# 2gunsu/monocon-pytorch

Hardware: AMD Instinct MI355X
Metric: images/sec (384x1280) fwd+bwd (higher is better)
Workload: dtype f32 (f16x2); 1 GPU; train step B=32/GPU 3x384x1280 (configs[2] shape, fp32 values, mode f16x2); global_batch=32, parallelism=dp1, precision_mode=f16x2

## Files before the change

### monocon-pytorch_amd/csrc/conv_bf16.hip

```cpp
#include "conv_mfma.h"

namespace mc {

typedef __bf16 bf16x8 __attribute__((ext_vector_type(8)));
typedef __bf16 bf16x4 __attribute__((ext_vector_type(4)));
typedef _Float16 f16x8 __attribute__((ext_vector_type(8)));
typedef _Float16 f16x4 __attribute__((ext_vector_type(4)));

template <int SPL> struct Piece { typedef __bf16 T; typedef bf16x8 V8; typedef bf16x4 V4; };
template <> struct Piece<2> { typedef _Float16 T; typedef f16x8 V8; typedef f16x4 V4; };
__device__ __forceinline__ f32x16 mfma_k16(bf16x8 a, bf16x8 b, f32x16 c) { return __builtin_amdgcn_mfma_f32_32x32x16_bf16(a, b, c, 0, 0, 0); }
__device__ __forceinline__ f32x16 mfma_k16(f16x8 a, f16x8 b, f32x16 c) { return __builtin_amdgcn_mfma_f32_32x32x16_f16(a, b, c, 0, 0, 0); }

template <int KS, int S, int WM, int WN, int WTM, int WTN, int SPL>
struct ConvCfgB16 {
    static constexpr int CK = 32;
    static constexpr int PB = WM * WTM, BNT = WN * WTN * 32, NT = 64 * WM * WN;
    static constexpr int KH = win_h(KS), KW = win_w(KS), PAD = win_pad(KS);
    static constexpr int IH = 3 * S + KH, IW = 7 * S + KW, NPIX = IH * IW;
    static constexpr int ROWB = (CK + 8) * 2;
    static constexpr bool PLANAR = S == 1;
    static constexpr int RS = 24;
    static constexpr int PPB = IH * RS * 16;
    static constexpr int CPL = ((PB + 1) / 2) * PPB + 32;
    static_assert(!PLANAR || (2 * IW <= RS && CK == 32), "two patches per 24-slot row, four 16-byte chunks per pixel");
    static constexpr int PLANE_BYTES = PLANAR ? 4 * CPL : PB * NPIX * ROWB;
    static constexpr int TILE_BYTES = SPL * PLANE_BYTES;
    static constexpr size_t LDS_BYTES = TILE_BYTES + PB * 16;
};

template <int KS, int S, int WM, int WN, int WTM, int WTN, int SPL, bool BM = false, bool LZ = false>
__global__ __launch_bounds__(64 * WM * WN, SPL == 1 ? 3 : 2) void conv_bf16_kernel(const ConvArgs a) {
    static_assert(!LZ || (SPL == 2 && !BM), "lazy sources: forward launches of the fp16-split mode");
    using Cfg = ConvCfgB16<KS, S, WM, WN, WTM, WTN, SPL>;
    typedef typename Piece<SPL>::T pc_t;
    typedef typename Piece<SPL>::V8 pc8;
    typedef typename Piece<SPL>::V4 pc4;
    constexpr int PLANE = Cfg::PLANE_BYTES;
    constexpr int CK = Cfg::CK, PB = Cfg::PB, BNT = Cfg::BNT, NT = Cfg::NT, PAD = Cfg::PAD;
    constexpr int IW = Cfg::IW, NPIX = Cfg::NPIX, ROWB = Cfg::ROWB;
    constexpr bool PLANAR = Cfg::PLANAR;
    constexpr int RS = Cfg::RS, PPB = Cfg::PPB, CPL = Cfg::CPL;
    constexpr int C4 = CK / 4;
    static_assert(NT % C4 == 0, "a thread keeps one channel group across its staging elements");

    extern __shared__ __attribute__((aligned(16))) unsigned char lds_raw[];
    int *pinfo = reinterpret_cast<int *>(lds_raw + Cfg::TILE_BYTES);

    const int tid = threadIdx.x;
    const int lane = tid & 63;
    const int wave = __builtin_amdgcn_readfirstlane(tid >> 6);
    const int wm = wave / WN, wn = wave % WN;
    const int g = lane >> 5, li = lane & 31;

    int img, chunk, n0;
    conv_wg<BNT>(a, img, chunk, n0);

    unsigned am_raw[4] = {0u, 0u, 0u, 0u};
    if constexpr (SPL == 2) {
        const int al = lane < AMAX_SUB ? lane * AMAX_STRIDE : 0;
#pragma unroll
        for (int i = 0; i < 4; ++i) am_raw[i] = a.amax_in[i < a.nsrc ? i : 0][al];
    }

    if (tid < PB) {
        const int pp = chunk * PB + tid;
        const int valid = pp < a.ppi;
        const int py = pp / a.ppr, px = pp % a.ppr;
        pinfo[tid * 4 + 0] = img;
        pinfo[tid * 4 + 1] = py * 4;
        pinfo[tid * 4 + 2] = px * 8;
        pinfo[tid * 4 + 3] = valid;
    }
    __syncthreads();

    float a_scale = 1.f, omul = 1.f;
    auto operand_scales = [&] {
        if constexpr (SPL == 2) {
            unsigned v = am_raw[0];
#pragma unroll
            for (int i = 1; i < 4; ++i) v = am_raw[i] > v ? am_raw[i] : v;
            v = lane < AMAX_SUB ? v : 0u;
#pragma unroll
            for (int o = 8; o > 0; o >>= 1) { const unsigned t = (unsigned)__shfl_xor((int)v, o); v = t > v ? t : v; }
            const int ea = f16_scale_exp((unsigned)__builtin_amdgcn_readfirstlane((int)v));
            const int ew = f16_scale_exp(*a.amax_w);
            a_scale = exp2i(ea);
            omul = exp2i(-ea) * exp2i(-ew);
        }
    };
    constexpr int NACC = SPL >= 2 ? 2 : 1;
    f32x16 acc[WTM][WTN], accm[NACC == 2 ? WTM : 1][NACC == 2 ? WTN : 1];
#pragma unroll
    for (int tm = 0; tm < WTM; ++tm)
#pragma unroll
        for (int tn = 0; tn < WTN; ++tn)
#pragma unroll
            for (int r = 0; r < 16; ++r) {
                acc[tm][tn][r] = 0.f;
                if (NACC == 2) accm[tm][tn][r] = 0.f;
            }

    constexpr int TOTAL = PB * NPIX * C4;
    constexpr int NIT = (TOTAL + NT - 1) / NT;
    const int c4 = tid % C4;
    unsigned char *stage_dst = lds_raw + (tid / C4) * ROWB + c4 * 8;

    int a_off[WTM];
#pragma unroll
    for (int tm = 0; tm < WTM; ++tm) {
        const int p = wm * WTM + tm;
        a_off[tm] = PLANAR ? g * CPL + (p >> 1) * PPB + ((li >> 3) * RS + (li & 7) + IW * (p & 1)) * 16
                           : (p * NPIX + ((li >> 3) * S) * IW + (li & 7) * S) * ROWB + g * 16;
    }

    const int Cin8 = a.Cin >> 3;
    const int w_plane = Cfg::KH * Cfg::KW * a.Cin * a.CoutP * 2;
    const __amdgpu_buffer_rsrc_t r_w = make_rsrc(a.wpk16, (unsigned)(SPL * w_plane));
    const int w_lane = (g * a.CoutP + n0 + wn * WTN * 32 + li) * 16;

    constexpr int KSTEPS = CK / 16, NS = Cfg::KH * Cfg::KW * KSTEPS;
    auto load_b = [&](pc8(&dst)[SPL][WTN], int kc, int s) {
        const int tap = s / KSTEPS, m = s % KSTEPS;
        const int soff = (tap * Cin8 + ((kc + m * 16) >> 3)) * a.CoutP * 16;
#pragma unroll
        for (int q = 0; q < SPL; ++q)
#pragma unroll
            for (int tn = 0; tn < WTN; ++tn)
                dst[q][tn] = __builtin_bit_cast(
                    pc8, __builtin_amdgcn_raw_buffer_load_b128(r_w, w_lane + tn * 32 * 16, soff + q * w_plane, 0));
    };
    auto load_a = [&](pc8(&dst)[SPL][WTM], int s) {
        const int tap = s / KSTEPS, m = s % KSTEPS;
#pragma unroll
        for (int q = 0; q < SPL; ++q)
#pragma unroll
            for (int tm = 0; tm < WTM; ++tm)
                dst[q][tm] = *reinterpret_cast<const pc8 *>(
                    lds_raw + q * PLANE + a_off[tm] +
                    (PLANAR ? 2 * m * CPL + ((tap / Cfg::KW) * RS + (tap % Cfg::KW)) * 16
                            : ((tap / Cfg::KW) * IW + (tap % Cfg::KW)) * ROWB + m * 32));
    };
#ifndef MC_CONV_DB_REGS
#define MC_CONV_DB_REGS 48
#endif
    constexpr int DB_FIT = MC_CONV_DB_REGS / (SPL * WTN * 4);
    constexpr int DB = (WTM * WTN > 2) ? 2 : ((DB_FIT >= 6 && NS % 6 == 0) ? 6 : ((DB_FIT >= 3 && NS % 3 == 0) ? 3 : 2));
    static_assert(NS % DB == 0, "ring slots must line up across K-chunks");
    pc8 bq[DB][SPL][WTN];
#pragma unroll
    for (int j = 0; j < DB - 1; ++j) load_b(bq[j], 0, j);
    const EpiCoef<WTN> coef = conv_epi_coef<WN, WTN, BM>(a, n0, wn, li);

#ifndef MC_CONV_PF
#define MC_CONV_PF 1
#endif
    constexpr bool PF = MC_CONV_PF && NIT <= 8 && WTM * WTN <= 2;
    constexpr int UB = NIT > 8 ? 8 : NIT;
    f32x4 pv[PF ? NIT : 1];
    int voff[NIT], sdst[NIT];
    int si = 0, c0 = 0, kc = 0;
    int Cs = a.src[0].C;
    f32x4 lzA = {0.f, 0.f, 0.f, 0.f}, lzB = lzA;
    bool lz_cur = false, lz_next = false;
    auto lazy_fetch = [&](int s_idx, int cc0) {
        if constexpr (LZ) {
            lz_next = a.src[s_idx].la != nullptr;
            if (lz_next) {
                lzA = reinterpret_cast<const f32x4 *>(a.src[s_idx].la + cc0)[c4];
                lzB = reinterpret_cast<const f32x4 *>(a.src[s_idx].lb + cc0)[c4];
            }
        }
    };
    auto lazy_advance = [&] {
        if constexpr (LZ) {
            lz_cur = lz_next;
            if (lz_cur) {
#pragma unroll
                for (int j = 0; j < 4; ++j) { lzA[j] *= a_scale; lzB[j] *= a_scale; }
            }
        }
    };
    __amdgpu_buffer_rsrc_t r_in = make_rsrc(a.src[0].p + (size_t)img * a.Hin * a.Win * Cs, (unsigned)(a.Hin * a.Win * Cs) * 4u);
    auto lane_offsets = [&](int cs) {
#pragma unroll
        for (int i = 0; i < NIT; ++i) {
            const int e = tid + NT * i;
            const int t = e / C4;
            const int pix = t % NPIX;
            const int p = (t / NPIX) % PB;
            const int iy = pix / IW, ix = pix % IW;
            const int y = pinfo[p * 4 + 1] * S - PAD + iy;
            const int x = pinfo[p * 4 + 2] * S - PAD + ix;
            const bool ok = (e < TOTAL) & (pinfo[p * 4 + 3] != 0) & ((unsigned)y < (unsigned)a.Hin) & ((unsigned)x < (unsigned)a.Win);
            int off = ((y * a.Win + x) * cs + c4 * 4) * 4;
            asm volatile("" : "+v"(off));
            voff[i] = ok ? off : BUF_OOB;
            sdst[i] = PLANAR ? (c4 >> 1) * CPL + (p >> 1) * PPB + (iy * RS + ix + IW * (p & 1)) * 16 + (c4 & 1) * 8
                             : (int)(stage_dst - lds_raw) + i * (NT / C4) * ROWB;
        }
    };
    auto stage_load = [&](__amdgpu_buffer_rsrc_t r, int vo, int so) -> f32x4 { return buf_load4(r, vo, so); };
    auto stage_one = [&](const f32x4 &v, int i, auto lz_c) {
        constexpr bool LZC = decltype(lz_c)::value;
        if (i < NIT && (NT * (i + 1) <= TOTAL || tid + NT * i < TOTAL)) {
            pc4 q[SPL];
            [[maybe_unused]] const float cap = voff[i] != BUF_OOB ? __builtin_inff() : 0.f;
#pragma unroll
            for (int j = 0; j < 4; ++j) {
                float r = SPL == 2 ? (LZC ? lazy_act(v[j], lzA[j], lzB[j], cap) : v[j] * a_scale) : v[j];
#pragma unroll
                for (int pz = 0; pz < SPL; ++pz) {
                    q[pz][j] = (pc_t)r;
                    r -= (float)q[pz][j];
                }
            }
#pragma unroll
            for (int pz = 0; pz < SPL; ++pz) *reinterpret_cast<pc4 *>(lds_raw + sdst[i] + pz * PLANE) = q[pz];
        }
    };
#ifdef MC_PHASE_TIMERS
    unsigned long long tp_stage = 0, tp_bar = 0, tp_mfma = 0, tp_epi = 0;
    const unsigned long long tp_t0 = __builtin_readcyclecounter();
#define TP_NOW() __builtin_readcyclecounter()
#else
#define TP_NOW() 0ull
#endif
    lane_offsets(Cs);
    lazy_fetch(0, 0);
    if (PF) {
#pragma unroll
        for (int i = 0; i < NIT; ++i) pv[i] = stage_load(r_in, voff[i], 0);
    }
    __builtin_amdgcn_sched_barrier(0);
    operand_scales();
    for (bool first = true;; first = false) {
        [[maybe_unused]] unsigned long long tp_a = TP_NOW();
        if (!first) __syncthreads();
        [[maybe_unused]] unsigned long long tp_b = TP_NOW();
        lazy_advance();
        auto stage_chunk = [&](auto lz_c) {
            if (PF) {
#pragma unroll
                for (int i = 0; i < NIT; ++i) stage_one(pv[i], i, lz_c);
            } else {
#pragma unroll
                for (int i0 = 0; i0 < NIT; i0 += UB) {
                    f32x4 v[UB];
#pragma unroll
                    for (int u = 0; u < UB; ++u)
                        if (i0 + u < NIT) v[u] = stage_load(r_in, voff[i0 + u], c0 * 4);
#pragma unroll
                    for (int u = 0; u < UB; ++u) stage_one(v[u], i0 + u, lz_c);
                }
            }
        };
        if constexpr (LZ) {
            if (lz_cur) stage_chunk(std::true_type{});
            else stage_chunk(std::false_type{});
        } else {
            stage_chunk(std::false_type{});
        }
        [[maybe_unused]] unsigned long long tp_c = TP_NOW();
        __syncthreads();
        [[maybe_unused]] unsigned long long tp_d = TP_NOW();
        int nsi = si, nc0 = c0 + CK;
        if (nc0 >= Cs) { ++nsi; nc0 = 0; }
        const bool more = nsi < a.nsrc;
        if (more && nsi != si) {
            Cs = a.src[nsi].C;
            r_in = make_rsrc(a.src[nsi].p + (size_t)img * a.Hin * a.Win * Cs, (unsigned)(a.Hin * a.Win * Cs) * 4u);
            lane_offsets(Cs);
        }
        if (more) lazy_fetch(nsi, nc0);
        if (PF && more) {
#pragma unroll
            for (int i = 0; i < NIT; ++i) pv[i] = stage_load(r_in, voff[i], nc0 * 4);
        }
        {
            const int kc_next = (kc + CK < a.Cin) ? kc + CK : kc;
            pc8 acur[SPL][WTM];
            load_a(acur, 0);
#pragma unroll
            for (int s = 0; s < NS; ++s) {
                pc8 anext[SPL][WTM];
                if (s + 1 < NS) load_a(anext, s + 1);
                {
                    const int t = s + DB - 1;
                    if (t < NS) load_b(bq[t % DB], kc, t);
                    else load_b(bq[t % DB], kc_next, t - NS);
                }
                __builtin_amdgcn_sched_barrier(0);
                constexpr int NP = SPL == 1 ? 1 : (SPL == 2 ? 3 : 6);
                constexpr int PA[6] = {SPL == 2 ? 1 : 0, SPL == 2 ? 0 : 2, SPL == 2 ? 0 : 1, 0, 1, 0};
                constexpr int PBv[6] = {SPL == 2 ? 0 : 2, SPL == 2 ? 1 : 0, SPL == 2 ? 0 : 1, 1, 0, 0};
#pragma unroll
                for (int pp = 0; pp < NP; ++pp)
#pragma unroll
                    for (int tm = 0; tm < WTM; ++tm)
#pragma unroll
                        for (int tn = 0; tn < WTN; ++tn) {
                            if (NACC == 2 && pp < NP - 1)
                                accm[tm][tn] = mfma_k16(acur[PA[pp]][tm], bq[s % DB][PBv[pp]][tn], accm[tm][tn]);
                            else
                                acc[tm][tn] = mfma_k16(acur[SPL == 1 ? 0 : PA[pp]][tm], bq[s % DB][SPL == 1 ? 0 : PBv[pp]][tn], acc[tm][tn]);
                        }
                if (s + 1 < NS) {
#pragma unroll
                    for (int q = 0; q < SPL; ++q)
#pragma unroll
                        for (int tm = 0; tm < WTM; ++tm) acur[q][tm] = anext[q][tm];
                }
            }
        }
#ifdef MC_PHASE_TIMERS
        { const unsigned long long tp_e = TP_NOW(); tp_bar += (tp_b - tp_a) + (tp_d - tp_c); tp_stage += tp_c - tp_b; tp_mfma += tp_e - tp_d; }
#endif
        if (!more) break;
        si = nsi; c0 = nc0; kc += CK;
    }
    [[maybe_unused]] const unsigned long long tp_f = TP_NOW();

    if (NACC == 2) {
#pragma unroll
        for (int tm = 0; tm < WTM; ++tm)
#pragma unroll
            for (int tn = 0; tn < WTN; ++tn)
#pragma unroll
                for (int r = 0; r < 16; ++r) acc[tm][tn][r] += accm[tm][tn][r];
    }
    conv_epilogue<WM, WN, WTM, WTN, BNT, BM>(a, acc, pinfo, chunk * PB, img, n0, wm, wn, g, li, coef, omul);
#ifdef MC_PHASE_TIMERS
    if (a.phase_prof && lane == 0) {
        __builtin_amdgcn_s_waitcnt(0);
        const unsigned long long tp_g = TP_NOW();
        tp_epi = tp_g - tp_f;
        unsigned long long *o = a.phase_prof + ((size_t)blockIdx.x * (NT / 64) + wave) * 5;
        o[0] = tp_stage; o[1] = tp_bar; o[2] = tp_mfma; o[3] = tp_epi; o[4] = tp_g - tp_t0;
    }
#endif
}

template <int KS, int S, class Sh, int SPL, bool BM = false, bool LZ = false>
static hipError_t launch_b16_one(ConvArgs a, hipStream_t st, ConvArgs *resolved) {
    using Cfg = ConvCfgB16<KS, S, Sh::WM, Sh::WN, Sh::WTM, Sh::WTN, SPL>;
    static_assert(Cfg::PB == Sh::PB && Cfg::BNT == Sh::BNT, "the shape table and the kernel agree on the tile");
    if constexpr (!LZ) {
        if (conv_any_lazy(a)) {
            if constexpr (SPL == 2 && !BM && (KS == 3 || KS == 1)) {
                if (a.bm_y) return hipErrorInvalidValue;
                return launch_b16_one<KS, S, Sh, SPL, false, true>(a, st, resolved);
            } else {
                return hipErrorInvalidValue;
            }
        }
    }
    if constexpr (!BM && S == 1 && (KS == 3 || KS == 1)) {
        if (a.bm_y) return launch_b16_one<KS, S, Sh, SPL, true>(a, st, resolved);
    } else if constexpr (!BM) {
        if (a.bm_y) return hipErrorInvalidValue;
    }
    conv_set_patches(a, Cfg::PB);
    if (a.CoutP % Cfg::BNT) return hipErrorInvalidValue;
    if (resolved) *resolved = a;
    return launch_dyn_lds<conv_bf16_kernel<KS, S, Sh::WM, Sh::WN, Sh::WTM, Sh::WTN, SPL, BM, LZ>>(
        Cfg::LDS_BYTES, dim3((unsigned)(a.B * a.chunks * (a.CoutP / Cfg::BNT))), dim3(Cfg::NT), st, a);
}

bool conv_bf16_ok(const ConvArgs &a, int ks, int stride) {
    if (!a.wpk16) return false;
    if (a.prec == 3) {
        if (!a.amax_w) return false;
        for (int i = 0; i < a.nsrc; ++i)
            if (!a.amax_in[i]) return false;
    }
    for (int i = 0; i < a.nsrc; ++i)
        if (a.src[i].C % 32) return false;
    if (ks == 3) return stride == 1 || stride == 2;
    return stride == 1 && (ks == 1 || ks == 12 || ks == 21 || ks == 22);
}

template <int SPL>
static hipError_t launch_conv_b16_spl(const ConvArgs &a, int ks, int stride, hipStream_t st, ConvArgs *resolved) {
    return with_conv_window(ks, stride, [&](auto win) {
        return with_conv_shape(a.cfg, [&](auto sh) {
            return launch_b16_one<decltype(win)::KS, decltype(win)::S, decltype(sh), SPL>(a, st, resolved);
        });
    });
}

hipError_t launch_conv_bf16(const ConvArgs &a, int ks, int stride, hipStream_t st, ConvArgs *resolved) {
    if (!conv_bf16_ok(a, ks, stride)) return hipErrorInvalidValue;
    if (a.prec == 3) return launch_conv_b16_spl<2>(a, ks, stride, st, resolved);
    return a.prec == 2 ? launch_conv_b16_spl<3>(a, ks, stride, st, resolved) : launch_conv_b16_spl<1>(a, ks, stride, st, resolved);
}

}
```

### monocon-pytorch_amd/csrc/conv_mfma.h

```cpp
#pragma once
#include <hip/hip_runtime.h>
#include <stdint.h>
#include <atomic>
#include <type_traits>
#include <utility>

namespace mc {

typedef float f32x16 __attribute__((ext_vector_type(16)));
typedef float f32x4 __attribute__((ext_vector_type(4)));

struct DynLdsOnce {
    std::atomic<unsigned long long> done{0};
    hipError_t ensure(const void *fn, int bytes) {
        int dev = 0;
        if (hipGetDevice(&dev) != hipSuccess || dev < 0 || dev >= 64) return hipFuncSetAttribute(fn, hipFuncAttributeMaxDynamicSharedMemorySize, bytes);
        if ((done.load(std::memory_order_acquire) >> dev) & 1ull) return hipSuccess;
        const hipError_t e = hipFuncSetAttribute(fn, hipFuncAttributeMaxDynamicSharedMemorySize, bytes);
        if (e == hipSuccess) done.fetch_or(1ull << dev, std::memory_order_release);
        return e;
    }
};

struct ConvSrc {
    const float *p;
    int C;
    const float *la, *lb;
};
__device__ __forceinline__ float lazy_act(float y, float a, float b, float cap) {
    return __builtin_amdgcn_fmed3f(__builtin_fmaf(y, a, b), 0.f, cap);
}

struct ConvArgs {
    ConvSrc src[4];
    int nsrc;
    int B, Hin, Win, Hout, Wout;
    int Cin;
    int Cout, CoutP;
    const float *wpk;
    const float *scale;
    const float *bias;
    const float *res;
    int res_ld;
    float *out;
    int out_ld, out_coff;
    int relu;
    float *stats;
    const float *stat_shift;
    int stats_centred;
    int ppr, ppi, chunks;
    int cfg;
    int o_img, o_row, o_px, r_img, r_row, r_px;
    const void *wpk16;
    int prec;
    const float *bm_y;
    const float *bm_z;
    const unsigned *bm_zbits;
    const float *bm_a, *bm_b;
    int bm_relu;
    const unsigned *amax_in[4];
    const unsigned *amax_w;
    unsigned *amax_out;
    unsigned long long *phase_prof;
};

__host__ __device__ __forceinline__ int f16_scale_exp(unsigned amax_bits) {
    const int E = (int)((amax_bits >> 23) & 0xffu);
    if (E == 0) return 0;
    const int e = 141 - E;
    return e > 126 ? 126 : e;
}
__host__ __device__ __forceinline__ float exp2i(int e) {
    const unsigned u = (unsigned)(127 + e) << 23;
    return __builtin_bit_cast(float, u);
}
constexpr int AMAX_SUB = 16, AMAX_STRIDE = 64, AMAX_WORDS = AMAX_SUB * AMAX_STRIDE;
__device__ __forceinline__ void amax_commit(unsigned *slot, unsigned bits) {
    unsigned *p = slot + (blockIdx.x % AMAX_SUB) * AMAX_STRIDE;
    if (bits < 0x7f800000u && bits > __hip_atomic_load(p, __ATOMIC_RELAXED, __HIP_MEMORY_SCOPE_AGENT)) atomicMax(p, bits);
}
__device__ __forceinline__ void amax_update_block(unsigned *slot, float v) {
    __shared__ unsigned s_amax;
    if (threadIdx.x == 0) s_amax = 0u;
    __syncthreads();
    const unsigned bits = __builtin_bit_cast(unsigned, v);
    if (bits < 0x7f800000u && bits != 0u) atomicMax(&s_amax, bits);
    __syncthreads();
    if (threadIdx.x == 0) amax_commit(slot, s_amax);
}
__device__ __forceinline__ void amax_update_wave(unsigned *slot, float v) {
#pragma unroll
    for (int o = 32; o > 0; o >>= 1) v = fmaxf(v, __shfl_xor(v, o));
    if ((threadIdx.x & 63) == 0) amax_commit(slot, __builtin_bit_cast(unsigned, v));
}
__device__ __forceinline__ unsigned amax_read(const unsigned *slot) {
    const int lane = threadIdx.x & 63;
    unsigned v = lane < AMAX_SUB ? slot[lane * AMAX_STRIDE] : 0u;
#pragma unroll
    for (int o = 8; o > 0; o >>= 1) { const unsigned t = (unsigned)__shfl_xor((int)v, o); v = t > v ? t : v; }
    return (unsigned)__builtin_amdgcn_readfirstlane((int)v);
}

constexpr int win_h(int ks) { return ks >= 10 ? ks / 10 : ks; }
constexpr int win_w(int ks) { return ks >= 10 ? ks % 10 : ks; }
constexpr int win_pad(int ks) { return ks == 3 ? 1 : 0; }

template <int KS, int S, int CK, int WM, int WN, int WTM, int WTN>
struct ConvCfg {
    static constexpr int PB = WM * WTM;
    static constexpr int BNT = WN * WTN * 32;
    static constexpr int NT = 64 * WM * WN;
    static constexpr int KH = win_h(KS), KW = win_w(KS);
    static constexpr int PAD = win_pad(KS);
    static constexpr int IH = 3 * S + KH;
    static constexpr int IW = 7 * S + KW;
    static constexpr int NPIX = IH * IW;
    static constexpr int CKP = CK + 4;
    static constexpr int LDS_FLOATS = PB * NPIX * CKP + PB * 4;
    static constexpr size_t LDS_BYTES = sizeof(float) * LDS_FLOATS;
};

constexpr int BUF_OOB = (int)0x80000000;
typedef int i32x4 __attribute__((ext_vector_type(4)));
__device__ __forceinline__ __amdgpu_buffer_rsrc_t make_rsrc(const void *base, unsigned bytes) {
    return __builtin_amdgcn_make_buffer_rsrc(const_cast<void *>(base), 0, (int)bytes, 0x00020000);
}
__device__ __forceinline__ f32x4 buf_load4(__amdgpu_buffer_rsrc_t r, int voff, int soff) {
    return __builtin_bit_cast(f32x4, __builtin_amdgcn_raw_buffer_load_b128(r, voff, soff, 0));
}
__device__ __forceinline__ float buf_load1(__amdgpu_buffer_rsrc_t r, int voff, int soff) {
    return __builtin_bit_cast(float, __builtin_amdgcn_raw_buffer_load_b32(r, voff, soff, 0));
}
__device__ __forceinline__ void buf_store1(float v, __amdgpu_buffer_rsrc_t r, int voff, int soff) {
    __builtin_amdgcn_raw_buffer_store_b32(__builtin_bit_cast(int, v), r, voff, soff, 0);
}

#ifndef MC_XCD_ORDER
#define MC_XCD_ORDER 1
#endif
__device__ __forceinline__ int xcd_order(int b, int n) {
    if (!MC_XCD_ORDER) return b;
    const int xcd = b & 7, idx = b >> 3, q = n >> 3, r = n & 7;
    return (xcd < r ? xcd * (q + 1) : r * (q + 1) + (xcd - r) * q) + idx;
}

template <int BNT>
__device__ __forceinline__ void conv_wg(const ConvArgs &a, int &img, int &chunk, int &n0) {
    const int ntiles = a.CoutP / BNT;
    const int bid = xcd_order(blockIdx.x, gridDim.x);
    const int nt = bid % ntiles;
    const int mchunk = bid / ntiles;
    img = mchunk / a.chunks, chunk = mchunk % a.chunks;
    n0 = nt * BNT;
}

template <int WTN>
struct EpiCoef {
    float sc[WTN], bi[WTN], sh[WTN], ma[WTN], mb[WTN];
};
template <int WN, int WTN, bool BM>
__device__ __forceinline__ EpiCoef<WTN> conv_epi_coef(const ConvArgs &a, int n0, int wn, int li) {
    EpiCoef<WTN> c;
#pragma unroll
    for (int tn = 0; tn < WTN; ++tn) {
        const int n = n0 + (wn * WTN + tn) * 32 + li;
        const bool nok = n < a.Cout;
        c.sc[tn] = (a.scale && nok) ? a.scale[n] : 1.f;
        c.bi[tn] = (a.bias && nok) ? a.bias[n] : 0.f;
        c.sh[tn] = (a.stat_shift && nok) ? a.stat_shift[n] : 0.f;
        c.ma[tn] = (BM && a.bm_relu == 2 && nok) ? a.bm_a[n] : 0.f;
        c.mb[tn] = (BM && a.bm_relu == 2 && nok) ? a.bm_b[n] : 0.f;
    }
    return c;
}

template <int WM, int WN, int WTM, int WTN, int BNT, bool BM = false>
__device__ __forceinline__ void conv_epilogue(const ConvArgs &a, f32x16 (&acc)[WTM][WTN], const int *pinfo,
                                              int patch0, int img, int n0, int wm, int wn, int g, int li,
                                              const EpiCoef<WTN> &coef, float omul = 1.f, float *vmax_acc = nullptr) {
#pragma clang fp contract(off)
    const bool do_stats = a.stats != nullptr;
    float vmax = 0.f;
    const bool has_res = a.res != nullptr;
    constexpr bool bm = BM;
    const int bm_relu = a.bm_relu;
    const float floor_v = a.relu ? 0.f : -__builtin_inff();
    const __amdgpu_buffer_rsrc_t r_out = make_rsrc(a.out + (size_t)img * a.o_img, (unsigned)a.o_img * 4u);
    const __amdgpu_buffer_rsrc_t r_res =
        make_rsrc(has_res ? a.res + (size_t)img * a.r_img : a.out, has_res ? (unsigned)a.r_img * 4u : 0u);
    const __amdgpu_buffer_rsrc_t r_y = make_rsrc(bm ? a.bm_y + (size_t)img * a.o_img : a.out, bm ? (unsigned)a.o_img * 4u : 0u);
    const bool zbits = bm && bm_relu == 1 && a.bm_zbits != nullptr;
    const int zwords = a.Cout >> 5;
    const unsigned zimg = zbits ? (unsigned)(a.Hout * a.Wout * zwords) * 4u : (unsigned)a.o_img * 4u;
    const __amdgpu_buffer_rsrc_t r_z =
        make_rsrc(bm && bm_relu == 1 ? (zbits ? reinterpret_cast<const float *>(a.bm_zbits) + (size_t)img * a.Hout * a.Wout * zwords
                                              : a.bm_z + (size_t)img * a.o_img)
                                     : a.out,
                  bm && bm_relu == 1 ? zimg : 0u);
#pragma unroll
    for (int tn = 0; tn < WTN; ++tn) {
        const int n = n0 + (wn * WTN + tn) * 32 + li;
        const bool nok = n < a.Cout;
        const float sc = coef.sc[tn] * omul, bi = coef.bi[tn], sh = coef.sh[tn], ma = coef.ma[tn], mb = coef.mb[tn];
        const int v_out = nok ? (4 * g * a.o_px + a.out_coff + n) * 4 : BUF_OOB;
        const int v_res = nok ? (4 * g * a.r_px + n) * 4 : BUF_OOB;
        const int v_bm = nok ? (4 * g * a.o_px + n) * 4 : BUF_OOB;
        const int v_zb = nok ? (4 * g * zwords + (n >> 5)) * 4 : BUF_OOB;
#pragma unroll
        for (int tm = 0; tm < WTM; ++tm) {
            const int p = wm * WTM + tm;
            const int oy0 = __builtin_amdgcn_readfirstlane(pinfo[p * 4 + 1]);
            const int ox0 = __builtin_amdgcn_readfirstlane(pinfo[p * 4 + 2]);
            const int pv = __builtin_amdgcn_readfirstlane(pinfo[p * 4 + 3]);
            if (!pv) continue;
            float ssum = 0.f, ssq = 0.f;
            if (oy0 + 4 <= a.Hout && ox0 + 8 <= a.Wout) {
                const int s_out = (oy0 * a.o_row + ox0 * a.o_px) * 4;
                const int s_res = (oy0 * a.r_row + ox0 * a.r_px) * 4;
                auto body = [&](auto res_c, auto zmask_c) {
                    constexpr bool RES = decltype(res_c)::value, ZMASK = decltype(zmask_c)::value;
                    float rv[16], yv[16], zv[16];
                    if constexpr (RES) {
#pragma unroll
                        for (int r = 0; r < 16; ++r)
                            rv[r] = buf_load1(r_res, v_res, s_res + ((r >> 2) * a.r_row + (r & 3) * a.r_px) * 4);
                    }
                    if constexpr (bm) {
#pragma unroll
                        for (int r = 0; r < 16; ++r)
                            yv[r] = buf_load1(r_y, v_bm, s_out + ((r >> 2) * a.o_row + (r & 3) * a.o_px) * 4);
                        if constexpr (ZMASK) {
                            if (zbits) {
                                const int s_zb = (oy0 * a.Wout + ox0) * zwords * 4;
#pragma unroll
                                for (int r = 0; r < 16; ++r) {
                                    const unsigned w = __builtin_bit_cast(unsigned, buf_load1(r_z, v_zb, s_zb + ((r >> 2) * a.Wout + (r & 3)) * zwords * 4));
                                    zv[r] = ((w >> (n & 31)) & 1u) ? 1.f : 0.f;
                                }
                            } else {
#pragma unroll
                                for (int r = 0; r < 16; ++r)
                                    zv[r] = buf_load1(r_z, v_bm, s_out + ((r >> 2) * a.o_row + (r & 3) * a.o_px) * 4);
                            }
                        }
                    }
#pragma unroll
                    for (int r = 0; r < 16; ++r) {
                        float v = __builtin_fmaf(acc[tm][tn][r], sc, bi);
                        if constexpr (RES) v += rv[r];
                        if constexpr (bm) {
                            const bool on = ZMASK ? zv[r] > 0.f : (bm_relu == 0 || fmaf(yv[r], ma, mb) > 0.f);
                            v = on ? v : 0.f;
                            ssum += v;
                            ssq = fmaf(v, yv[r], ssq);
                        } else if (do_stats) {
                            const float d = v - sh;
                            ssum += d;
                            ssq += d * d;
                        }
                        v = fmaxf(v, floor_v);
                        vmax = fmaxf(vmax, fabsf(v));
                        buf_store1(v, r_out, v_out, s_out + ((r >> 2) * a.o_row + (r & 3) * a.o_px) * 4);
                    }
                };
                using T = std::true_type;
                using Fz = std::false_type;
                const bool zmask = bm && bm_relu == 1;
                if (has_res) { if (zmask) body(T{}, T{}); else body(T{}, Fz{}); }
                else { if (zmask) body(Fz{}, T{}); else body(Fz{}, Fz{}); }
            } else {
#pragma unroll
                for (int r = 0; r < 16; ++r) {
                    const int y = oy0 + (r >> 2), x = ox0 + (r & 3) + 4 * g;
                    if (nok && y < a.Hout && x < a.Wout) {
                        float v = __builtin_fmaf(acc[tm][tn][r], sc, bi);
                        if (has_res) v += buf_load1(r_res, (y * a.r_row + x * a.r_px + n) * 4, 0);
                        if (bm) {
                            const float yy = buf_load1(r_y, (y * a.o_row + x * a.o_px + n) * 4, 0);
                            bool on = true;
                            if (bm_relu == 1)
                                on = zbits ? ((__builtin_bit_cast(unsigned, buf_load1(r_z, ((y * a.Wout + x) * zwords + (n >> 5)) * 4, 0)) >> (n & 31)) & 1u) != 0u
                                           : buf_load1(r_z, (y * a.o_row + x * a.o_px + n) * 4, 0) > 0.f;
                            else if (bm_relu == 2) on = fmaf(yy, ma, mb) > 0.f;
                            v = on ? v : 0.f;
                            ssum += v;
                            ssq = fmaf(v, yy, ssq);
                        } else {
                            const float d = v - sh;
                            ssum += d;
                            ssq += d * d;
                        }
                        v = fmaxf(v, floor_v);
                        vmax = fmaxf(vmax, fabsf(v));
                        buf_store1(v, r_out, (y * a.o_row + x * a.o_px + a.out_coff + n) * 4, 0);
                    }
                }
            }
            if (do_stats) {
                ssum += __shfl_xor(ssum, 32);
                if constexpr (!bm) {
                    if (a.stats_centred) {
                        const float m = ssum * 0.03125f;
                        ssq = 0.f;
#pragma unroll
                        for (int r = 0; r < 16; ++r) {
                            const float e = (__builtin_fmaf(acc[tm][tn][r], sc, bi) - sh) - m;
                            ssq = __builtin_fmaf(e, e, ssq);
                        }
                    }
                }
                ssq += __shfl_xor(ssq, 32);
                if (g == 0 && nok) {
                    float *dst = a.stats + (((size_t)img * a.ppi + patch0 + p) * a.CoutP + n) * 2;
                    dst[0] = ssum;
                    dst[1] = ssq;
                }
            }
        }
    }
    if (vmax_acc) *vmax_acc = fmaxf(*vmax_acc, vmax);
    else if (a.amax_out) amax_update_wave(a.amax_out, vmax);
}

enum ConvCfgId {
    CFG_AUTO = 0,
    CFG_128x128 = 1,
    CFG_128x64 = 4,
    CFG_128x64m = 5,
    CFG_128x32 = 6,
    CFG_64x128 = 7,
    CFG_64x64 = 8,
    CFG_SHAPE_BITS = 15,
    CFG_WS = 16,
    CFG_SMALL = 32,
    CFG_WRES = 64
};
struct ConvShape {
    int id, WM, WN, WTM, WTN;
    constexpr int PB() const { return WM * WTM; }
    constexpr int BNT() const { return WN * WTN * 32; }
};
constexpr ConvShape CONV_SHAPES[] = {
    {CFG_128x128, 2, 2, 2, 2}, {CFG_128x64, 2, 2, 2, 1}, {CFG_128x64m, 4, 1, 1, 2},
    {CFG_128x32, 4, 1, 1, 1},  {CFG_64x128, 1, 4, 2, 1}, {CFG_64x64, 2, 2, 1, 1},
};
constexpr int CONV_NSHAPES = (int)(sizeof(CONV_SHAPES) / sizeof(CONV_SHAPES[0]));
inline ConvShape conv_shape(int cfg) {
    for (const ConvShape &s : CONV_SHAPES)
        if (s.id == (cfg & CFG_SHAPE_BITS)) return s;
    return {0, 0, 0, 0, 0};
}
// ... 91 lines not shown
```

### monocon-pytorch_amd/csrc/mc_api.hip

```cpp
#include <hip/hip_runtime.h>

#include <algorithm>
#include <cmath>
#include <cstdarg>
#include <cstdio>
#include <cstring>
#include <cstdlib>
#include <map>
#include <memory>
#include <string>
#include <unordered_map>
#include <vector>

#include "../../include/monocon_hip.h"
#include "conv_mfma.h"
#include "kernels.h"

#include <cstdint>
#include "mc_internal.h"

std::string g_create_err;

float *PlanAlloc::alloc(size_t nfloats) {
    const size_t bytes = (nfloats ? nfloats : empty_floats) * sizeof(float);
// ... 922 lines not shown

int mc_op_stem_dgrad_fused(mc_handle *h, const float *d_nhwc, const float *y_nhwc, const float *coef, const float *weight_oihw,
                           int B, int H, int W, float *dx_nchw, void *stream) {
    if (!h) return -1;
    if (!d_nhwc || !y_nhwc || !coef || !weight_oihw || !dx_nchw) return fail(h, "mc_op_stem_dgrad_fused: null argument");
    if (B < 1 || H < 1 || W < 1) return fail(h, "mc_op_stem_dgrad_fused: B, H, W must be >= 1 (got %d, %d, %d)", B, H, W);
    if (reinterpret_cast<uintptr_t>(d_nhwc) % 16 || reinterpret_cast<uintptr_t>(y_nhwc) % 16 || reinterpret_cast<uintptr_t>(coef) % 16)
        return fail(h, "mc_op_stem_dgrad_fused: d_nhwc, y_nhwc and coef must be 16-byte aligned");
    HIPCHK(h, hipSetDevice(h->device));
    HIPCHK(h, launch_stem_dgrad(d_nhwc, weight_oihw, B, H, W, dx_nchw, static_cast<hipStream_t>(stream), y_nhwc, coef));
    return 0;
}

int mc_op_maxpool2(mc_handle *h, const float *in, int B, int H, int W, int C, float *out, void *stream) {
    if (!h) return -1;
    if (!in || !out || (C % 4) || (H % 2) || (W % 2)) return fail(h, "mc_op_maxpool2: bad argument");
    HIPCHK(h, hipSetDevice(h->device));
    HIPCHK(h, launch_maxpool2(in, B, H, W, C, out, static_cast<hipStream_t>(stream)));
    return 0;
}

int mc_op_deconv4x4(mc_handle *h, const float *in, int B, int H, int W, int C, const float *weight, float *out,
                    void *stream) {
    if (!h) return -1;
    if (!in || !out || !weight || (C % 4)) return fail(h, "mc_op_deconv4x4: bad argument");
    HIPCHK(h, hipSetDevice(h->device));
    hipStream_t st = static_cast<hipStream_t>(stream);
    ScratchBuf wpk;
    HIPCHK(h, wpk.alloc((size_t)16 * C * sizeof(float)));
    HIPCHK(h, launch_pack_deconv_w(weight, C, wpk.as<float>(), st));
    hipError_t e = launch_deconv4(in, B, H, W, C, wpk.as<float>(), out, st);
    hipError_t e2 = hipStreamSynchronize(st);
    HIPCHK(h, e);
    HIPCHK(h, e2);
    return 0;
}

int mc_op_nchw_to_nhwc(mc_handle *h, const float *in, int B, int C, int H, int W, float *out, void *stream) {
    if (!h) return -1;
    if (!in || !out) return fail(h, "mc_op_nchw_to_nhwc: null argument");
    HIPCHK(h, hipSetDevice(h->device));
    HIPCHK(h, launch_nchw_to_nhwc(in, B, C, H, W, out, static_cast<hipStream_t>(stream)));
    return 0;
}

int mc_op_nhwc_to_nchw(mc_handle *h, const float *in, int B, int C, int H, int W, float *out, void *stream) {
    if (!h) return -1;
    if (!in || !out) return fail(h, "mc_op_nhwc_to_nchw: null argument");
    HIPCHK(h, hipSetDevice(h->device));
    HIPCHK(h, launch_nhwc_to_nchw(in, B, C, H, W, out, static_cast<hipStream_t>(stream)));
    return 0;
}

int mc_preprocess(mc_handle *h, const void *img_hwc, int dtype, int H, int W, const double mean[3], const double std[3],
                  int pad_h, int pad_w, float *out_chw, void *stream) {
    if (!h) return -1;
    if (!img_hwc || !mean || !std || !out_chw) return fail(h, "mc_preprocess: null argument");
    if (dtype != 0 && dtype != 2) return fail(h, "mc_preprocess: dtype must be 0 (float32) or 2 (uint8)");
    if (H < 1 || W < 1 || pad_h < H || pad_w < W) return fail(h, "mc_preprocess: bad shape %dx%d -> %dx%d", H, W, pad_h, pad_w);
    for (int c = 0; c < 3; ++c)
        if (std[c] == 0.0) return fail(h, "mc_preprocess: std[%d] is zero", c);
    HIPCHK(h, hipSetDevice(h->device));
    HIPCHK(h, launch_preprocess(img_hwc, dtype == 2, H, W, mean, std, pad_h, pad_w, out_chw, static_cast<hipStream_t>(stream)));
    return 0;
}

int mc_preprocess_augmented(mc_handle *h, const unsigned char *frames_hwc, const float *params, int B, int src_h, int src_w,
                            const double mean[3], const double std[3], int pad_h, int pad_w, float *out_bchw, void *stream) {
    if (!h) return -1;
    if (!frames_hwc || !params || !mean || !std || !out_bchw) return fail(h, "mc_preprocess_augmented: null argument");
    if (B < 1 || src_h < 1 || src_w < 1 || pad_h < 1 || pad_w < 1 || B > 65535 || pad_h > 65535)
        return fail(h, "mc_preprocess_augmented: bad shape B=%d %dx%d -> %dx%d", B, src_h, src_w, pad_h, pad_w);
    for (int c = 0; c < 3; ++c)
        if (std[c] == 0.0) return fail(h, "mc_preprocess_augmented: std[%d] is zero", c);
    HIPCHK(h, hipSetDevice(h->device));
    HIPCHK(h, launch_preprocess_aug(frames_hwc, params, B, src_h, src_w, mean, std, pad_h, pad_w, out_bchw, static_cast<hipStream_t>(stream)));
    return 0;
}

int mc_bench_mfma_peak(mc_handle *h, int waves_per_simd, int iters, float *tflops) {
    if (!h || !tflops) return fail(h, "mc_bench_mfma_peak: null argument");
    HIPCHK(h, hipSetDevice(h->device));
    void *out = nullptr;
    HIPCHK(h, hipMalloc(&out, 64));
    hipEvent_t e0, e1;
    HIPCHK(h, hipEventCreate(&e0));
    HIPCHK(h, hipEventCreate(&e1));
    const int blocks = 256 * (waves_per_simd < 0 ? -waves_per_simd : waves_per_simd);
    hipLaunchKernelGGL(mfma_peak_kernel, dim3(blocks), dim3(256), 0, nullptr, (float *)out, 100, waves_per_simd < 0 ? -1.0f : 1.0f);
    (void)hipEventRecord(e0, nullptr);
    hipLaunchKernelGGL(mfma_peak_kernel, dim3(blocks), dim3(256), 0, nullptr, (float *)out, iters, waves_per_simd < 0 ? -1.0f : 1.0f);
    (void)hipEventRecord(e1, nullptr);
    (void)hipEventSynchronize(e1);
    float ms = 0;
    (void)hipEventElapsedTime(&ms, e0, e1);
    *tflops = (float)((double)blocks * 4 * iters * 16 * 4096.0 / (ms * 1e-3) / 1e12);
    (void)hipEventDestroy(e0);
    (void)hipEventDestroy(e1);
    (void)hipFree(out);
    return 0;
}

int mc_bench_conv(mc_handle *h, int B, int Hin, int Win, int nsrc, const int src_channels[], int Cout, int ksize,
                  int stride, int cfg, int iters, float *ms_avg) {
    if (!h || !src_channels || !ms_avg) return fail(h, "mc_bench_conv: null argument");
    HIPCHK(h, hipSetDevice(h->device));
    ConvArgs a{};
    std::vector<void *> bufs;
    const bool zero_data = std::getenv("MONOCON_BENCH_ZERO") != nullptr;
    auto alloc_fill = [&](size_t n, float scale) -> float * {
        if (zero_data) scale = 0.f;
        void *q = nullptr;
        if (hipMalloc(&q, n * sizeof(float)) != hipSuccess) return nullptr;
        bufs.push_back(q);
        std::vector<float> hst(std::min<size_t>(n, (size_t)1 << 22));
        unsigned s = 12345u + (unsigned)bufs.size();
        for (auto &v : hst) { s = s * 1664525u + 1013904223u; v = scale * (((s >> 8) & 0xFFFF) / 32768.0f - 1.0f); }
        for (size_t off = 0; off < n; off += hst.size())
            (void)hipMemcpy((float *)q + off, hst.data(), std::min(hst.size(), n - off) * sizeof(float), hipMemcpyHostToDevice);
        return (float *)q;
    };
    Tensor x[4];
    std::vector<const Tensor *> xs;
    ConvLayer L;
    L.ks = ksize; L.stride = stride; L.cout = Cout; L.coutp = conv_coutp(Cout);
    for (int i = 0; i < nsrc; ++i) {
        x[i] = operand_tensor(alloc_fill((size_t)B * Hin * Win * src_channels[i], 1.0f), B, Hin, Win, src_channels[i]);
        if (!x[i].p) return fail(h, "mc_bench_conv: out of memory");
        xs.push_back(&x[i]);
        L.cin += src_channels[i];
    }
    const int Ho = conv_out_dim(Hin, ksize, stride), Wo = conv_out_dim(Win, ksize, stride);
    const size_t wn = fwd_panel_elems(ksize, L.cin, L.coutp), on = (size_t)B * Ho * Wo * Cout;
    const size_t stats_n = (size_t)B * conv_chunks_per_image(CFG_AUTO, Ho, Wo) * L.coutp * 2;
    L.wpk = alloc_fill(wn, 0.05f);
    a.scale = alloc_fill(Cout, 1.0f);
    a.bias = alloc_fill(Cout, 1.0f);
    a.out = alloc_fill(on, 0.0f);
    if (!L.wpk || !a.scale || !a.bias || !a.out) return fail(h, "mc_bench_conv: out of memory");
    a.out_ld = Cout; a.relu = 1; a.cfg = cfg;
    if (const char *e = std::getenv("MONOCON_BENCH_STATS")) {
        if (std::atoi(e)) a.stats = alloc_fill(stats_n, 0.f);
    }
    if (const char *e = std::getenv("MONOCON_BENCH_BM")) {
        const int m = std::atoi(e);
        if (m) {
            a.relu = 0;
            a.stats = alloc_fill(stats_n, 0.f);
            a.bm_y = alloc_fill(on, 1.0f);
            a.bm_a = a.scale; a.bm_b = a.bias; a.bm_relu = m == 1 ? 2 : 1;
            if (m >= 2) a.bm_z = alloc_fill(on, 1.0f);
            if (m >= 3) { a.res = alloc_fill(on, 1.0f); a.res_ld = Cout; }
            if (!a.stats || !a.bm_y || (m >= 2 && !a.bm_z) || (m >= 3 && !a.res)) return fail(h, "mc_bench_conv: out of memory");
        }
    }
    if (h->prec >= 1 && L.cin % 32 == 0) {
        std::vector<unsigned short> hw(wn * 3);
        unsigned s16 = 777u;
        for (auto &v : hw) { s16 = s16 * 1664525u + 1013904223u; v = zero_data ? 0 : (unsigned short)(0x2c00u + ((s16 >> 12) & 0x3ffu) + ((s16 >> 31) << 15)); }
        void *q = nullptr;
        if (hipMalloc(&q, hw.size() * 2) != hipSuccess) return fail(h, "mc_bench_conv: out of memory");
        bufs.push_back(q);
        (void)hipMemcpy(q, hw.data(), hw.size() * 2, hipMemcpyHostToDevice);
        L.wpk16 = q;
        std::vector<unsigned> one((size_t)5 * AMAX_WORDS, 0x3f800000u);
        if (hipMalloc(&q, one.size() * 4) != hipSuccess) return fail(h, "mc_bench_conv: out of memory");
        bufs.push_back(q);
        (void)hipMemcpy(q, one.data(), one.size() * 4, hipMemcpyHostToDevice);
        for (int i = 0; i < nsrc; ++i) x[i].amax = static_cast<unsigned *>(q) + (size_t)i * AMAX_WORDS;
        L.w_amax = static_cast<unsigned *>(q) + (size_t)4 * AMAX_WORDS;
    }
    conv_fwd_args(a, L, xs, h->prec);
#ifdef MC_PHASE_TIMERS
    const size_t prof_n = (size_t)1 << 22;
    {
        void *q = nullptr;
        if (hipMalloc(&q, prof_n * 8) != hipSuccess) return fail(h, "mc_bench_conv: out of memory");
        bufs.push_back(q);
        (void)hipMemset(q, 0, prof_n * 8);
        a.phase_prof = static_cast<unsigned long long *>(q);
    }
#endif
    hipEvent_t e0, e1;
    HIPCHK(h, hipEventCreate(&e0));
    HIPCHK(h, hipEventCreate(&e1));
    hipError_t e = launch_conv(a, ksize, stride, nullptr);
    if (e == hipSuccess) e = launch_conv(a, ksize, stride, nullptr);
    if (e == hipSuccess) {
        (void)hipEventRecord(e0, nullptr);
        for (int i = 0; i < iters && e == hipSuccess; ++i) e = launch_conv(a, ksize, stride, nullptr);
        (void)hipEventRecord(e1, nullptr);
        (void)hipEventSynchronize(e1);
        float ms = 0;
        (void)hipEventElapsedTime(&ms, e0, e1);
        *ms_avg = ms / iters;
#ifdef MC_PHASE_TIMERS
        if (a.phase_prof) {
            std::vector<unsigned long long> hp(prof_n);
            (void)hipMemcpy(hp.data(), a.phase_prof, prof_n * 8, hipMemcpyDeviceToHost);
            double sum[5] = {0, 0, 0, 0, 0};
            size_t n = 0;
            for (size_t i = 0; i + 5 <= prof_n; i += 5)
                if (hp[i + 4]) { for (int k = 0; k < 5; ++k) sum[k] += (double)hp[i + k]; ++n; }
            if (n) std::fprintf(stderr, "[phase] waves %zu  avg cycles per wave: stage %.0f  barriers %.0f  mfma-phase %.0f  epilogue %.0f  total %.0f\n",
                                n, sum[0] / n, sum[1] / n, sum[2] / n, sum[3] / n, sum[4] / n);
        }
#endif
    }
    (void)hipEventDestroy(e0);
    (void)hipEventDestroy(e1);
    for (void *q : bufs) (void)hipFree(q);
    HIPCHK(h, e);
    return 0;
}

int mc_set_conv_cfg(mc_handle *h, int cfg) {
    if (!h) return -1;
    const int shape_bits = cfg & CFG_SHAPE_BITS;
    if (cfg != CFG_SMALL && (cfg < 0 || (shape_bits && !conv_shape(cfg).id) || (cfg & ~(CFG_SHAPE_BITS | CFG_WS | CFG_WRES))))
        return fail(h, "mc_set_conv_cfg: unknown shape id");
    if ((cfg & (CFG_WS | CFG_WRES)) && !shape_bits) return fail(h, "mc_set_conv_cfg: the kernel-variant flags need a shape");
    h->force_cfg = cfg;
    HIPCHK(h, hipSetDevice(h->device));
    HIPCHK(h, hipDeviceSynchronize());
    for (auto &kv : h->plans) kv.second->mem.release();
    h->plans.clear();
    return 0;
}

int mc_tune_export(mc_handle *h, int *buf, int cap, int *n_ints) {
    if (!h || !n_ints) return -1;
    int n = 0;
    for (auto &kv : h->tuned) n += 2 + (int)kv.first.size();
    *n_ints = n;
    if (!buf) return 0;
    if (cap < n) return fail(h, "mc_tune_export: buffer of %d ints, %d needed", cap, n);
    int o = 0;
    for (auto &kv : h->tuned) {
        buf[o++] = (int)kv.first.size();
        for (int v : kv.first) buf[o++] = v;
        buf[o++] = kv.second;
    }
    return 0;
}

int mc_tune_import(mc_handle *h, const int *buf, int n_ints) {
    if (!h || (!buf && n_ints > 0)) return -1;
    std::vector<std::pair<std::vector<int>, int>> entries;
    int o = 0;
    while (o < n_ints) {
        const int kl = buf[o++];
        if (kl < 10 || kl > 16 || o + kl + 1 > n_ints) return fail(h, "mc_tune_import: malformed table at int %d", o - 1);
        std::vector<int> key(buf + o, buf + o + kl);
        o += kl;
        const int cfg = buf[o++];
        if (cfg != CFG_SMALL && (cfg <= 0 || !conv_shape(cfg).id || (cfg & ~(CFG_SHAPE_BITS | CFG_WS | CFG_WRES))))
            return fail(h, "mc_tune_import: unknown shape id %d", cfg);
        const int bnt = cfg == CFG_SMALL ? 0 : conv_shape(cfg).BNT();
        if (cfg != CFG_SMALL && (bnt <= 0 || key[6] <= 0 || key[6] % bnt))
            return fail(h, "mc_tune_import: the %d-column tile of shape id %d does not divide CoutP = %d of its entry", bnt, cfg, key[6]);
        entries.emplace_back(std::move(key), cfg);
    }
    for (auto &e : entries) h->tuned[e.first] = e.second;
    return (int)entries.size();
}

int mc_set_local_maximum_kernel(mc_handle *h, int kernel) {
    if (!h) return -1;
    if (kernel < 1 || kernel > 31 || kernel % 2 == 0)
        return fail(h, "mc_set_local_maximum_kernel: the window must be odd, 1 .. 31 (got %d)", kernel);
    h->lm_kernel = kernel;
    return 0;
}

int mc_set_precision(mc_handle *h, int mode) {
    if (!h) return -1;
    if (mode < 0 || mode > 3)
        return fail(h, "mc_set_precision: mode must be 0 (fp32 MFMA), 1 (bf16 MFMA operands), 2 (fp32 emulated by a 3-way bf16 "
                       "split) or 3 (fp32 emulated by a 2-way fp16 split)");
    if (mode == h->prec) return 0;
    HIPCHK(h, hipSetDevice(h->device));
    HIPCHK(h, hipDeviceSynchronize());
    h->prec = mode;
    for (auto &kv : h->plans) kv.second->mem.release();
    h->plans.clear();
    h->bind_gen++;
    h->pack_clean = false;
    h->packed = false;
    return 0;
}

int mc_train_query_workspace(mc_handle *h, int B, int H, int W, int head_only, size_t *bytes);

int mc_query_workspace(mc_handle *h, int B, int H, int W, int mode, size_t *bytes) {
    if (!h || !bytes) return -1;
    if (B < 1 || H < 32 || W < 32 || (H % 32) || (W % 32)) return fail(h, "mc_query_workspace: B >= 1, H and W multiples of 32");
    if (mode == 0) {
        if (!h->packed) return fail(h, "mc_query_workspace: bind all parameters and call mc_pack_params first");
        auto it = h->plans.find(std::make_tuple(B, H, W));
        if (it != h->plans.end()) { *bytes = it->second->mem.bytes; return 0; }
        h->dry_alloc = true; h->dry_next = 0;
        (void)get_plan(h, B, H, W);
        h->dry_alloc = false;
        *bytes = h->dry_next;
        return *bytes ? 0 : -1;
    }
// ... 75 lines not shown
```

Baseline: 671.7 images/sec.

## Software-pipeline the conv epilogue's residual and mask loads across tiles

Adds a pipelined path to the conv epilogue for selected f16-split kernel shapes. When residual or backward-mask inputs are present and all patches in the wave are fully in bounds, it prefetches the residual, y and mask values for the next tile into a double buffer while the current tile is scaled, masked and stored. The goal is to hide global-load latency in the memory-bound epilogue, at the cost of more registers, more template instantiations and a duplicated code path. The benchmark helper also gains options for a bit-packed mask and a residual input.

```diff
diff --git a/monocon-pytorch_amd/csrc/conv_bf16.hip b/monocon-pytorch_amd/csrc/conv_bf16.hip
--- a/monocon-pytorch_amd/csrc/conv_bf16.hip
+++ b/monocon-pytorch_amd/csrc/conv_bf16.hip
@@ -28,6 +28,10 @@
     static constexpr int TILE_BYTES = SPL * PLANE_BYTES;
     static constexpr size_t LDS_BYTES = TILE_BYTES + PB * 16;
 };
+
+template <int KS, int S, int WTM, int WTN, int SPL, bool BM, bool LZ>
+constexpr bool EPI_PIPE_B16 = epi_pipe_shape(WTM, WTN) && SPL >= 2 &&
+                              (WTM * WTN == 2 || (SPL == 2 && S == 1 && !LZ && (KS == 1 || (KS == 3 && !BM))));
 
 template <int KS, int S, int WM, int WN, int WTM, int WTN, int SPL, bool BM = false, bool LZ = false>
 __global__ __launch_bounds__(64 * WM * WN, SPL == 1 ? 3 : 2) void conv_bf16_kernel(const ConvArgs a) {
@@ -329,7 +333,7 @@
 #pragma unroll
                 for (int r = 0; r < 16; ++r) acc[tm][tn][r] += accm[tm][tn][r];
     }
-    conv_epilogue<WM, WN, WTM, WTN, BNT, BM>(a, acc, pinfo, chunk * PB, img, n0, wm, wn, g, li, coef, omul);
+    conv_epilogue<WM, WN, WTM, WTN, BNT, BM, EPI_PIPE_B16<KS, S, WTM, WTN, SPL, BM, LZ>>(a, acc, pinfo, chunk * PB, img, n0, wm, wn, g, li, coef, omul);
 #ifdef MC_PHASE_TIMERS
     if (a.phase_prof && lane == 0) {
         __builtin_amdgcn_s_waitcnt(0);
diff --git a/monocon-pytorch_amd/csrc/conv_mfma.h b/monocon-pytorch_amd/csrc/conv_mfma.h
--- a/monocon-pytorch_amd/csrc/conv_mfma.h
+++ b/monocon-pytorch_amd/csrc/conv_mfma.h
@@ -174,7 +174,12 @@
     return c;
 }
 
-template <int WM, int WN, int WTM, int WTN, int BNT, bool BM = false>
+#ifndef MC_EPI_PIPE
+#define MC_EPI_PIPE 1
+#endif
+constexpr bool epi_pipe_shape(int WTM, int WTN) { return MC_EPI_PIPE && WTM * WTN > 1 && WTM <= 2; }
+
+template <int WM, int WN, int WTM, int WTN, int BNT, bool BM = false, bool PIPE = false>
 __device__ __forceinline__ void conv_epilogue(const ConvArgs &a, f32x16 (&acc)[WTM][WTN], const int *pinfo,
                                               int patch0, int img, int n0, int wm, int wn, int g, int li,
                                               const EpiCoef<WTN> &coef, float omul = 1.f, float *vmax_acc = nullptr) {
@@ -197,6 +202,145 @@
                                               : a.bm_z + (size_t)img * a.o_img)
                                      : a.out,
                   bm && bm_relu == 1 ? zimg : 0u);
+    if constexpr (PIPE) {
+        static_assert(WTM <= 2 && WTM * WTN > 1, "see epi_pipe_shape()");
+        int oyv[WTM], oxv[WTM], nv = 0;
+        bool uniform = true;
+#pragma unroll
+        for (int tm = 0; tm < WTM; ++tm) {
+            const int p = wm * WTM + tm;
+            oyv[tm] = __builtin_amdgcn_readfirstlane(pinfo[p * 4 + 1]);
+            oxv[tm] = __builtin_amdgcn_readfirstlane(pinfo[p * 4 + 2]);
+            if (__builtin_amdgcn_readfirstlane(pinfo[p * 4 + 3])) {
+                if (oyv[tm] + 4 <= a.Hout && oxv[tm] + 8 <= a.Wout && nv == tm) ++nv;
+                else uniform = false;
+            }
+        }
+        if ((bm || has_res) && uniform && (nv == WTM || (WTN > 1 && nv == 1))) {
+            auto walk = [&](auto nv_c, auto res_c, auto zmask_c) __attribute__((always_inline)) {
+                constexpr int NV = decltype(nv_c)::value, NTP = NV * WTN;
+                constexpr bool RES = decltype(res_c)::value;
+                constexpr int ZM = decltype(zmask_c)::value;
+                float rv[2][16], yv[2][16], zv[2][16];
+                unsigned zw[2];
+                int vo_out[WTN], vo_res[WTN], vo_bm[WTN], vo_zb[WTN];
+#pragma unroll
+                for (int tn = 0; tn < WTN; ++tn) {
+                    const int n = n0 + (wn * WTN + tn) * 32 + li;
+                    const bool nok = n < a.Cout;
+                    vo_out[tn] = nok ? (4 * g * a.o_px + a.out_coff + n) * 4 : BUF_OOB;
+                    vo_res[tn] = nok ? (4 * g * a.r_px + n) * 4 : BUF_OOB;
+                    vo_bm[tn] = nok ? (4 * g * a.o_px + n) * 4 : BUF_OOB;
+                    vo_zb[tn] = nok ? ((((li >> 2) & 3) * a.Wout + 4 * g + (li & 3)) * zwords + (n >> 5)) * 4 : BUF_OOB;
+                }
+#pragma unroll
+                for (int u = 0; u <= NTP; ++u) {
+                    if (u < NTP) {
+                        const int tn = u / NV, tm = u % NV, set = u & 1;
+                        const int v_res = vo_res[tn], v_bm = vo_bm[tn], v_zb = vo_zb[tn];
+                        const int s_out = (oyv[tm] * a.o_row + oxv[tm] * a.o_px) * 4;
+                        const int s_res = (oyv[tm] * a.r_row + oxv[tm] * a.r_px) * 4;
+                        if constexpr (RES) {
+#pragma unroll
+                            for (int r = 0; r < 16; ++r)
+                                rv[set][r] = buf_load1(r_res, v_res, s_res + ((r >> 2) * a.r_row + (r & 3) * a.r_px) * 4);
+                        }
+                        if constexpr (bm) {
+#pragma unroll
+                            for (int r = 0; r < 16; ++r)
+                                yv[set][r] = buf_load1(r_y, v_bm, s_out + ((r >> 2) * a.o_row + (r & 3) * a.o_px) * 4);
+                            if constexpr (ZM == 2) {
+                                zw[set] = __builtin_bit_cast(unsigned, buf_load1(r_z, v_zb, (oyv[tm] * a.Wout + oxv[tm]) * zwords * 4));
+                            } else if constexpr (ZM == 1) {
+#pragma unroll
+                                for (int r = 0; r < 16; ++r)
+                                    zv[set][r] = buf_load1(r_z, v_bm, s_out + ((r >> 2) * a.o_row + (r & 3) * a.o_px) * 4);
+                            }
+                        }
+                    }
+                    __builtin_amdgcn_sched_barrier(0);
+                    if (u > 0) {
+                        const int tn = (u - 1) / NV, tm = (u - 1) % NV, set = (u - 1) & 1;
+                        const int p = wm * WTM + tm;
+                        const int n = n0 + (wn * WTN + tn) * 32 + li;
+                        const bool nok = n < a.Cout;
+                        const float sc = coef.sc[tn] * omul, bi = coef.bi[tn], sh = coef.sh[tn], ma = coef.ma[tn], mb = coef.mb[tn];
+                        const int v_out = vo_out[tn];
+                        const int s_out = (oyv[tm] * a.o_row + oxv[tm] * a.o_px) * 4;
+                        float ssum = 0.f, ssq = 0.f;
+#pragma unroll
+                        for (int r = 0; r < 16; ++r) {
+                            float v = __builtin_fmaf(acc[tm][tn][r], sc, bi);
+                            if constexpr (RES) v += rv[set][r];
+                            if constexpr (bm) {
+                                bool on;
+                                if constexpr (ZM == 2) {
+                                    const unsigned w0 = (unsigned)__builtin_amdgcn_readlane((int)zw[set], r);
+                                    const unsigned w1 = (unsigned)__builtin_amdgcn_readlane((int)zw[set], 32 + r);
+                                    on = (((g ? w1 : w0) >> (n & 31)) & 1u) != 0u;
+                                } else if constexpr (ZM == 1) {
+                                    on = zv[set][r] > 0.f;
+                                } else {
+                                    on = bm_relu == 0 || fmaf(yv[set][r], ma, mb) > 0.f;
+                                }
+                                v = on ? v : 0.f;
+                                ssum += v;
+                                ssq = fmaf(v, yv[set][r], ssq);
+                            } else if (do_stats) {
+                                const float d = v - sh;
+                                ssum += d;
+                                ssq += d * d;
+                            }
+                            v = fmaxf(v, floor_v);
+                            vmax = fmaxf(vmax, fabsf(v));
+                            buf_store1(v, r_out, v_out, s_out + ((r >> 2) * a.o_row + (r & 3) * a.o_px) * 4);
+                        }
+                        if (do_stats) {
+                            ssum += __shfl_xor(ssum, 32);
+                            if constexpr (!bm) {
+                                if (a.stats_centred) {
+                                    const float m = ssum * 0.03125f;
+                                    ssq = 0.f;
+#pragma unroll
+                                    for (int r = 0; r < 16; ++r) {
+                                        const float e = (__builtin_fmaf(acc[tm][tn][r], sc, bi) - sh) - m;
+                                        ssq = __builtin_fmaf(e, e, ssq);
+                                    }
+                                }
+                            }
+                            ssq += __shfl_xor(ssq, 32);
+                            if (g == 0 && nok) {
+                                float *dst = a.stats + (((size_t)img * a.ppi + patch0 + p) * a.CoutP + n) * 2;
+                                dst[0] = ssum;
+                                dst[1] = ssq;
+                            }
+                        }
+                    }
+                }
+            };
+            using T = std::true_type;
+            using Fz = std::false_type;
+            using Z0 = std::integral_constant<int, 0>;
+            using Z1 = std::integral_constant<int, 1>;
+            using Z2 = std::integral_constant<int, 2>;
+            auto by_patches = [&](auto res_c, auto zmask_c) __attribute__((always_inline)) {
+                if constexpr (WTM > 1 && WTN > 1) {
+                    if (nv < WTM) { walk(std::integral_constant<int, 1>{}, res_c, zmask_c); return; }
+                }
+                walk(std::integral_constant<int, WTM>{}, res_c, zmask_c);
+            };
+            if constexpr (bm) {
+                const int zm = bm_relu == 1 ? (zbits ? 2 : 1) : 0;
+                if (has_res) { if (zm == 2) by_patches(T{}, Z2{}); else if (zm == 1) by_patches(T{}, Z1{}); else by_patches(T{}, Z0{}); }
+                else { if (zm == 2) by_patches(Fz{}, Z2{}); else if (zm == 1) by_patches(Fz{}, Z1{}); else by_patches(Fz{}, Z0{}); }
+            } else {
+                by_patches(T{}, Z0{});
+            }
+            if (vmax_acc) *vmax_acc = fmaxf(*vmax_acc, vmax);
+            else if (a.amax_out) amax_update_wave(a.amax_out, vmax);
+            return;
+        }
+    }
 #pragma unroll
     for (int tn = 0; tn < WTN; ++tn) {
         const int n = n0 + (wn * WTN + tn) * 32 + li;
diff --git a/monocon-pytorch_amd/csrc/mc_api.hip b/monocon-pytorch_amd/csrc/mc_api.hip
--- a/monocon-pytorch_amd/csrc/mc_api.hip
+++ b/monocon-pytorch_amd/csrc/mc_api.hip
@@ -1098,6 +1098,24 @@
             if (m >= 2) a.bm_z = alloc_fill(on, 1.0f);
             if (m >= 3) { a.res = alloc_fill(on, 1.0f); a.res_ld = Cout; }
             if (!a.stats || !a.bm_y || (m >= 2 && !a.bm_z) || (m >= 3 && !a.res)) return fail(h, "mc_bench_conv: out of memory");
+            if (m == 4) {
+                if (Cout % 32) return fail(h, "mc_bench_conv: a bit-packed mask needs Cout % 32 == 0");
+                const size_t words = on / 32;
+                void *q = nullptr;
+                if (hipMalloc(&q, words * 4) != hipSuccess) return fail(h, "mc_bench_conv: out of memory");
+                bufs.push_back(q);
+                std::vector<unsigned> hz(std::min<size_t>(words, (size_t)1 << 22));
+                unsigned s = 4242u;
+                for (auto &v : hz) { s = s * 1664525u + 1013904223u; v = zero_data ? 0u : (s ^ (s >> 15)); }
+                for (size_t off = 0; off < words; off += hz.size())
+                    (void)hipMemcpy((unsigned *)q + off, hz.data(), std::min(hz.size(), words - off) * 4, hipMemcpyHostToDevice);
+                a.bm_zbits = static_cast<const unsigned *>(q);
+            }
+        }
+    } else if (const char *e = std::getenv("MONOCON_BENCH_RES")) {
+        if (std::atoi(e)) {
+            a.res = alloc_fill(on, 1.0f); a.res_ld = Cout;
+            if (!a.res) return fail(h, "mc_bench_conv: out of memory");
         }
     }
     if (h->prec >= 1 && L.cin % 32 == 0) {
```

New measurement: 673.7 images/sec (median of 6 runs). Within noise of the previous version (+0.3%).
